# BichenWuUCB/squeezeDet

Hardware: AMD Instinct MI355X
Metric: images/sec SqueezeDet 1242x375 inference (higher is better)
Workload: dtype f16; 1 GPU; squeezeDet fp16 inference, batch=32 per GPU, synthetic 1242x375 images (4 distinct batches in rotation), full hot path (forward + interpret_output + filter_prediction + filtered rows to pinned host memory), inputs resident in HBM; 2 batches in flight (consecutive steps alternate between 2 HIP streams); global_batch=32, parallelism=dp1 (independent image shards, no collective)

## Files before the change

squeezedet_amd/csrc/chain.hip:

```cpp
#include "conv_common.h"
#include "chain.h"
#include "filter_body.h"

namespace sqdet {

namespace {

constexpr int CROWS = 8, CCOLS = 16;
constexpr int CHP = (CROWS + 2) * (CCOLS + 2);
constexpr int CCHUNK = CHP * 64;
constexpr int STAGE_B = 12288;
constexpr int NIMG = 2;

struct ChainGeom {
  int nch, nsq, nb1, nb3, chain, base3, per3, nstages;
};

__host__ __device__ inline ChainGeom chain_geom(int s, int e1, int e3, int s2) {
  ChainGeom g;
  g.nch = (s * 2 + 63) / 64;
  g.nsq = s2 / 16;
  g.nb1 = e1 / 64;
  g.nb3 = e3 / 64;
  g.chain = s2 > 0 ? 1 : 0;
  g.base3 = g.nb1 * (1 + g.chain);
  g.per3 = 3 * g.nch + g.chain;
  g.nstages = g.base3 + g.nb3 * g.per3;
  return g;
}

struct ChainArgs {
  const void* sq_in;
  void* sq_out;
  void* y;
  const unsigned char* stream;
  const float *b1, *b3, *bs2;
  int N, H, W, S, E1, E3, S2;
  int tiles_x, tiles_y;
  int nb1, nb3, nstages;
  unsigned in_bytes, out_bytes, y_bytes;
  int per_xcd;
  ChainRide ride;
};

__device__ __forceinline__ void glds16(unsigned voff, const unsigned char* sbase, unsigned lds_dst) {
  asm volatile("s_mov_b32 m0, %2\n\ts_nop 0\n\tglobal_load_lds_dwordx4 %0, %1" ::"v"(voff), "s"(sbase), "s"(lds_dst) : "memory", "m0");
}

#ifdef SQDET_CHAIN_TIMELINE
__device__ unsigned long long g_chain_tl[4096 * 8];
#define CTL(k) do { ctl[k] = wall_clock64(); } while (0)
#else
#define CTL(k) do {} while (0)
#endif

template <int N>
__device__ __forceinline__ void vm_wait() {
  asm volatile("s_waitcnt vmcnt(%0)" ::"n"(N) : "memory");
}

__device__ __forceinline__ i32x4 pack8(const f32x4& a, const f32x4& b) {
  f16x8 h = {(f16)a[0], (f16)a[1], (f16)a[2], (f16)a[3], (f16)b[0], (f16)b[1], (f16)b[2], (f16)b[3]};
  return __builtin_bit_cast(i32x4, h);
}

__device__ __forceinline__ f32x4 relu4(f32x4 v) {
  v[0] = fmaxf(v[0], 0.f); v[1] = fmaxf(v[1], 0.f); v[2] = fmaxf(v[2], 0.f); v[3] = fmaxf(v[3], 0.f);
  return v;
}

template <int NCH, int NSQ, bool WY, int RING, int DBG = 0>
__global__ __launch_bounds__(512, 2) void fire_chain(ChainArgs a) {
  using T = f16;
  constexpr int LOOK = RING - 2;
  constexpr int TH = (NSQ + 1) / 2;
  extern __shared__ __attribute__((aligned(16))) unsigned char lds[];
  const int lane = threadIdx.x & 63;
  const int wave = __builtin_amdgcn_readfirstlane((int)(threadIdx.x >> 6));
  const int pg = wave & 3, h = wave >> 2;
  const int j = lane & 15, g = lane >> 4;
#ifdef SQDET_CHAIN_TIMELINE
  unsigned long long ctl[8] = {0, 0, 0, 0, 0, 0, 0, 0};
#endif
  CTL(0);

  if ((int)(blockIdx.x >> 3) >= a.per_xcd) {
    const int rider = (int)((blockIdx.x >> 3) - a.per_xcd) * 8 + (int)(blockIdx.x & 7);
    FastLds<512>& fs = *reinterpret_cast<FastLds<512>*>(lds);
    for (int im = rider; im < a.ride.nimg; im += a.ride.nriders) {
      filter_one_image<true, f16, 512>(a.ride.fa, a.ride.da, a.ride.img0 + im, fs);
      __syncthreads();
    }
    return;
  }
  int b = (int)((blockIdx.x & 7) * a.per_xcd + (blockIdx.x >> 3));
  const int npairs = (a.N + 1) >> 1;
  if (b >= npairs * a.tiles_x * a.tiles_y) return;
  const int tx = b % a.tiles_x; b /= a.tiles_x;
  const int ty = b % a.tiles_y;
  const int np = b / a.tiles_y;
  const int oy0 = ty * CROWS, ox0 = tx * CCOLS;

  unsigned char* ring = lds;
  unsigned char* stile = lds + RING * STAGE_B;
  unsigned char* xch = stile + NIMG * NCH * CCHUNK;
  float* bl = reinterpret_cast<float*>(xch + (NSQ > 0 ? 32768 : 0));
  const unsigned ring_addr = (unsigned)(uintptr_t)(__attribute__((address_space(3))) unsigned char*)ring;

  constexpr int NP = NCH * 4;
  constexpr int SIT = (NIMG * CHP * NP + 511) / 512;
  i32x4 sv[SIT];
  {
    const int s_pieces = a.S * 2 / 16;
    const __amdgpu_buffer_rsrc_t rin = __builtin_amdgcn_make_buffer_rsrc(const_cast<void*>(a.sq_in), 0, a.in_bytes, 0x00020000);
    constexpr unsigned OOB = 0xfffffff0u;
#pragma unroll
    for (int it = 0; it < SIT; ++it) {
      const int idx = it * 512 + (int)threadIdx.x;
      const int im = idx / (CHP * NP);
      const int rem = idx - im * (CHP * NP);
      const int P = rem / NP, q = rem - P * NP;
      const int r = P / (CCOLS + 2), c = P - r * (CCOLS + 2);
      const int iy = oy0 - 1 + r, ix = ox0 - 1 + c;
      const int n = np * 2 + im;
      const bool ok = idx < NIMG * CHP * NP && q < s_pieces && n < a.N && iy >= 0 && iy < a.H && ix >= 0 && ix < a.W;
      const unsigned off = ok ? (unsigned)((((n * a.H + iy) * a.W + ix) * a.S) * 2 + q * 16) : OOB;
      sv[it] = __builtin_amdgcn_raw_buffer_load_b128(rin, off, 0, 0);
    }
  }

  const unsigned voff1 = (unsigned)(wave * 1024 + lane * 16), voff2 = voff1 + 8192;
  const unsigned char* sp = a.stream;
  const unsigned m0_lo = ring_addr + (unsigned)wave * 1024;
  unsigned m0n = m0_lo;
  auto refill = [&]() {
    if constexpr (DBG >= 2) return;
    glds16(voff1, sp, m0n);
    if (h == 0) glds16(voff2, sp, m0n + 8192);
    sp += STAGE_B;
    m0n = m0n + STAGE_B == m0_lo + RING * STAGE_B ? m0_lo : m0n + STAGE_B;
  };
#pragma unroll
  for (int s = 0; s < LOOK; ++s) refill();
  CTL(1);

  {
#pragma unroll
    for (int it = 0; it < SIT; ++it) {
      const int idx = it * 512 + (int)threadIdx.x;
      const int im = idx / (CHP * NP);
      const int rem = idx - im * (CHP * NP);
      const int P = rem / NP, q = rem - P * NP;
      if (idx < NIMG * CHP * NP)
        *reinterpret_cast<i32x4*>(stile + (im * NCH + (q >> 2)) * CCHUNK + P * 64 + (((q & 3) ^ ((P >> 1) & 3)) << 4)) = sv[it];
    }
    const int nbias = a.E1 + a.E3 + a.S2;
    for (int i = threadIdx.x; i < nbias; i += 512)
      bl[i] = i < a.E1 ? a.b1[i] : (i < a.E1 + a.E3 ? a.b3[i - a.E1] : a.bs2[i - a.E1 - a.E3]);
  }
  __syncthreads();
  CTL(2);

  const int img = pg >> 1, r0 = (pg & 1) * 4;
  const unsigned char* simg = stile + img * NCH * CCHUNK;
  auto load_b = [&](int c, int rr, int dx) {
    const int P = (r0 + rr) * (CCOLS + 2) + j + dx;
    return *reinterpret_cast<const i32x4*>(simg + c * CCHUNK + P * 64 + ((g ^ ((P >> 1) & 3)) << 4));
  };
  unsigned cbo = 0, nbo = STAGE_B;
  auto lda = [&](unsigned bo, int f) {
    return *reinterpret_cast<const i32x4*>(ring + bo + f * 1024 + lane * 16);
  };
  int ks = 0, ep_ks = -100;
  auto sync = [&](bool lds_writes) {
    bool st = false;
    if constexpr (WY) { st = (ks - ep_ks) < LOOK; ++ks; }
    if constexpr (DBG < 1) {
      if (h == 0) { if (st) vm_wait<2 * (LOOK - 1) + 4>(); else vm_wait<2 * (LOOK - 1)>(); }
      else { if (st) vm_wait<(LOOK - 1) + 4>(); else vm_wait<(LOOK - 1)>(); }
    }
    if (lds_writes) asm volatile("s_waitcnt lgkmcnt(0)" ::: "memory");
    if constexpr (DBG < 3) __builtin_amdgcn_s_barrier();
    asm volatile("" ::: "memory");
  };
  auto next_buf = [&]() {
    cbo = nbo;
    nbo = nbo + STAGE_B == RING * STAGE_B ? 0 : nbo + STAGE_B;
  };

  f32x4 accs[TH > 0 ? TH : 1][4];
#pragma unroll
  for (int t = 0; t < (TH > 0 ? TH : 1); ++t)
#pragma unroll
    for (int m = 0; m < 4; ++m) accs[t][m] = f32x4{0.f, 0.f, 0.f, 0.f};

  const int ctot = a.E1 + a.E3;
  const __amdgpu_buffer_rsrc_t ry = __builtin_amdgcn_make_buffer_rsrc(a.y, 0, WY ? a.y_bytes : 0u, 0x00020000);
  const int n_img = np * 2 + img;
  const int ox = ox0 + j;
  const bool col_ok = ox < a.W && n_img < a.N;

  i32x4 an[2];
  sync(false);
  CTL(3);
  refill();
#pragma unroll
  for (int n = 0; n < 2; ++n) an[n] = lda(0, 2 * h + n);

  auto finish_block = [&](f32x4 (&acc)[4][2], int cc0) {
    i32x4 bf[4];
    {
      const f32x4 bias0 = *reinterpret_cast<const f32x4*>(bl + cc0 + h * 32 + g * 8);
      const f32x4 bias1 = *reinterpret_cast<const f32x4*>(bl + cc0 + h * 32 + g * 8 + 4);
#pragma unroll
      for (int m = 0; m < 4; ++m) bf[m] = pack8(relu4(acc[m][0] + bias0), relu4(acc[m][1] + bias1));
    }
    if (WY) {
#pragma unroll
      for (int m = 0; m < 4; ++m) {
        const int oy = oy0 + r0 + m;
        const bool ok = col_ok && oy < a.H;
        const unsigned off = ok ? (unsigned)((((n_img * a.H + oy) * a.W + ox) * ctot + cc0 + h * 32 + g * 8) * 2) : 0xfffffff0u;
        __builtin_amdgcn_raw_buffer_store_b128(bf[m], ry, off, 0, 0);
      }
      ep_ks = ks;
    }
    if constexpr (NSQ > 0) {
      i32x4 fr[2][TH];
#pragma unroll
      for (int u = 0; u < 2; ++u)
#pragma unroll
        for (int i = 0; i < TH; ++i) {
          const int t = min(h * TH + i, NSQ - 1);
          fr[u][i] = lda(cbo, u * NSQ + t);
        }
#pragma unroll
      for (int m = 0; m < 4; ++m)
        *reinterpret_cast<i32x4*>(xch + (wave * 4 + m) * 1024 + lane * 16) = bf[m];
      sync(true);
      i32x4 bx[2][4];
#pragma unroll
      for (int u = 0; u < 2; ++u)
#pragma unroll
        for (int m = 0; m < 4; ++m) bx[u][m] = *reinterpret_cast<const i32x4*>(xch + ((pg + 4 * u) * 4 + m) * 1024 + lane * 16);
#pragma unroll
      for (int n = 0; n < 2; ++n) an[n] = lda(nbo, 2 * h + n);
#pragma unroll
      for (int u = 0; u < 2; ++u) {
#pragma unroll
        for (int i = 0; i < TH; ++i) {
          if (NSQ % 2 == 0 || h * TH + i < NSQ) {
#pragma unroll
            for (int m = 0; m < 4; ++m) mma16<T>(accs[i][m], fr[u][i], bx[u][m]);
          }
          if (u == 0 && i == 0) refill();
        }
      }
      next_buf();
    }
  };

  {
    i32x4 b1f[NCH][4];
#pragma unroll
    for (int c = 0; c < NCH; ++c)
#pragma unroll
      for (int m = 0; m < 4; ++m) b1f[c][m] = load_b(c, m + 1, 1);
#pragma unroll 1
    for (int blk = 0; blk < a.nb1; ++blk) {
      f32x4 acc[4][2];
#pragma unroll
      for (int m = 0; m < 4; ++m)
#pragma unroll
        for (int n = 0; n < 2; ++n) acc[m][n] = f32x4{0.f, 0.f, 0.f, 0.f};
      i32x4 ac[2];
#pragma unroll
      for (int n = 0; n < 2; ++n) ac[n] = an[n];
#pragma unroll
      for (int c = 0; c < NCH; ++c) {
        i32x4 nx[2];
        if (c + 1 < NCH) {
#pragma unroll
          for (int n = 0; n < 2; ++n) nx[n] = lda(cbo, (c + 1) * 4 + 2 * h + n);
        } else {
          sync(false);
#pragma unroll
          for (int n = 0; n < 2; ++n) nx[n] = lda(nbo, 2 * h + n);
        }
#pragma unroll
        for (int m = 0; m < 4; ++m) {
#pragma unroll
          for (int n = 0; n < 2; ++n) mma16<T>(acc[m][n], ac[n], b1f[c][m]);
          if (c + 1 == NCH && m == 2 * h) refill();
        }
#pragma unroll
        for (int n = 0; n < 2; ++n) ac[n] = nx[n];
      }
#pragma unroll
      for (int n = 0; n < 2; ++n) an[n] = ac[n];
      next_buf();
      finish_block(acc, blk * 64);
    }
  }

  CTL(4);
  i32x4 B[6][3];
#pragma unroll
  for (int rr = 0; rr < 2; ++rr)
#pragma unroll
    for (int dx = 0; dx < 3; ++dx) B[rr][dx] = load_b(0, rr, dx);
#pragma unroll 1
  for (int blk = 0; blk < a.nb3; ++blk) {
    f32x4 acc[4][2];
#pragma unroll
    for (int m = 0; m < 4; ++m)
#pragma unroll
      for (int n = 0; n < 2; ++n) acc[m][n] = f32x4{0.f, 0.f, 0.f, 0.f};
    i32x4 ac[2];
#pragma unroll
    for (int n = 0; n < 2; ++n) ac[n] = an[n];
#pragma unroll
    for (int c = 0; c < NCH; ++c) {
#pragma unroll
      for (int dy = 0; dy < 3; ++dy) {
        if (DBG >= 4 && blk > 0) {
        } else if (dy == 0) {
#pragma unroll
          for (int rr = 2; rr < 5; ++rr)
#pragma unroll
            for (int dx = 0; dx < 3; ++dx) B[rr][dx] = load_b(c, rr, dx);
        } else if (dy == 1) {
#pragma unroll
          for (int dx = 0; dx < 3; ++dx) B[5][dx] = load_b(c, 5, dx);
        } else {
#pragma unroll
          for (int rr = 0; rr < 2; ++rr)
#pragma unroll
            for (int dx = 0; dx < 3; ++dx) B[rr][dx] = load_b((c + 1) % NCH, rr, dx);
        }
#pragma unroll
        for (int dx = 0; dx < 3; ++dx) {
          i32x4 nx[2];
          if (DBG >= 5 && blk > 0) {
            nx[0] = ac[1]; nx[1] = ac[0];
            if (dx == 2) sync(false);
          } else if (dx < 2) {
#pragma unroll
            for (int n = 0; n < 2; ++n) nx[n] = lda(cbo, (dx + 1) * 4 + 2 * h + n);
          } else {
            sync(false);
#pragma unroll
            for (int n = 0; n < 2; ++n) nx[n] = lda(nbo, 2 * h + n);
          }
#pragma unroll
          for (int m = 0; m < 4; ++m) {
#pragma unroll
            for (int n = 0; n < 2; ++n) mma16<T>(acc[m][n], ac[n], B[m + dy][dx]);
            if (dx == 2 && m == 2 * h) refill();
          }
#pragma unroll
          for (int n = 0; n < 2; ++n) ac[n] = nx[n];
        }
        next_buf();
      }
    }
#pragma unroll
    for (int n = 0; n < 2; ++n) an[n] = ac[n];
    if constexpr (DBG >= 6) {
#pragma unroll
      for (int m = 0; m < 4; ++m)
#pragma unroll
        for (int n = 0; n < 2; ++n) accs[0][m] += acc[m][n];
      next_buf();
    } else {
      finish_block(acc, a.E1 + blk * 64);
    }
  }
  CTL(5);
  vm_wait<0>();
  CTL(6);

  if constexpr (NSQ > 0) {
    T* so = reinterpret_cast<T*>(a.sq_out);
    const float* bs = bl + a.E1 + a.E3;
#pragma unroll
    for (int m = 0; m < 4; ++m) {
      const int oy = oy0 + r0 + m;
      if (col_ok && oy < a.H) {
        T* dst = so + ((size_t)(n_img * a.H + oy) * a.W + ox) * a.S2 + g * 4 * NSQ;
#pragma unroll
        for (int i = 0; i < TH; ++i) {
          const int t = h * TH + i;
          if (t < NSQ) {
            const f32x4 bias = *reinterpret_cast<const f32x4*>(bs + g * 4 * NSQ + t * 4);
            store4<T>(dst + t * 4, relu4(accs[i][m] + bias));
          }
        }
      }
    }
  }
#ifdef SQDET_CHAIN_TIMELINE
  CTL(7);
  if (threadIdx.x == 0 && blockIdx.x < 4096) {
#pragma unroll
    for (int k = 0; k < 8; ++k) g_chain_tl[(size_t)blockIdx.x * 8 + k] = ctl[k];
  }
#endif
}

__global__ void chain_pack_kernel(const float* __restrict__ w1, const float* __restrict__ w3, const float* __restrict__ ws2,
                                  f16* __restrict__ out, int S, int E1, int E3, int S2, ChainGeom gm, size_t total) {
  for (size_t idx = (size_t)blockIdx.x * blockDim.x + threadIdx.x; idx < total; idx += (size_t)gridDim.x * blockDim.x) {
    size_t t = idx;
    const int e = t % 8; t /= 8;
    const int lane = t % 64; t /= 64;
    const int tile = t % 4; t /= 4;
    const int slot = t % 3; t /= 3;
    const int stage = (int)t;
    const int i = lane & 15, g = lane >> 4;
    int kind, blk, r;
    int cc0 = 0;
    if (stage < gm.base3) {
      blk = stage / (1 + gm.chain);
      r = stage - blk * (1 + gm.chain);
      kind = r == 0 ? 0 : 2;
      cc0 = blk * 64;
    } else {
      const int k2 = stage - gm.base3;
      blk = k2 / gm.per3;
      r = k2 - blk * gm.per3;
      kind = r < 3 * gm.nch ? 1 : 2;
      cc0 = E1 + blk * 64;
    }
    const float* src = kind == 0 ? w1 : (kind == 1 ? w3 : ws2);
    if (!src) continue;
    float v = 0.f;
    if (kind == 2) {
      const int f = slot * 4 + tile;
      if (f < 2 * gm.nsq) {
        const int u = f / gm.nsq, tt = f - u * gm.nsq;
        const int co = (i >> 2) * 4 * gm.nsq + tt * 4 + (i & 3);
        const int ci = cc0 + u * 32 + g * 8 + e;
        v = ws2[(size_t)ci * S2 + co];
      }
    } else {
      const int co = blk * 64 + (tile >> 1) * 32 + (i >> 2) * 8 + (tile & 1) * 4 + (i & 3);
      if (kind == 0) {
        const int ci = slot * 32 + g * 8 + e;
        if (slot < gm.nch && ci < S) v = w1[(size_t)ci * E1 + co];
      } else {
        const int c = r / 3, dy = r - c * 3;
        const int ci = c * 32 + g * 8 + e;
        if (ci < S) v = w3[((size_t)(dy * 3 + slot) * S + ci) * E3 + co];
      }
    }
    out[idx] = (f16)v;
  }
}

struct ChainSArgs {
  const void* sq_in;
  void* sq_out;
  const unsigned char* stream;
  const float *b1, *b3, *bs2;
  int N, H, W, S, E1, E3, S2;
  int tiles_x, tiles_y, ntiles, nquads;
  int nb1, nb3;
  unsigned in_bytes;
};

constexpr int CS_TILES = 4;
constexpr int CS_LW = 24;
constexpr int CS_TILE_B = (CROWS + 2) * CS_LW * 64;

template <int NSQ>
__global__ __launch_bounds__(512, 2) void fire_chain_stream(ChainSArgs a) {
  using T = f16;
  constexpr int F1 = 4 + 2 * NSQ;
  constexpr int F3 = 36 + 2 * NSQ;
  constexpr int NP = 4;
  constexpr int SIT = (CHP * NP + 127) / 128;
  extern __shared__ __attribute__((aligned(16))) unsigned char lds[];
  const int lane = threadIdx.x & 63;
  const int wave = __builtin_amdgcn_readfirstlane((int)(threadIdx.x >> 6));
  const int j = lane & 15, g = lane >> 4;
  const int nfrag = a.nb1 * F1 + a.nb3 * F3;
  unsigned char* wres = lds;
  unsigned char* stile = lds + (size_t)nfrag * 1024;
  float* bl = reinterpret_cast<float*>(stile + CS_TILES * CS_TILE_B);

// ... 135 lines not shown
#pragma unroll
      for (int m = 0; m < 4; ++m) Bc[m] = load_b(m, 0);
#pragma unroll
      for (int tt = 0; tt < 4; ++tt) ac[tt] = wfrag(f0 + tt);
#pragma unroll
      for (int tap = 0; tap < 9; ++tap) {
        i32x4 Bn[4], an[4];
        if (tap + 1 < 9) {
          const int dy = (tap + 1) / 3, dx = (tap + 1) % 3;
#pragma unroll
          for (int m = 0; m < 4; ++m) Bn[m] = load_b(m + dy, dx);
#pragma unroll
          for (int tt = 0; tt < 4; ++tt) an[tt] = wfrag(f0 + (tap + 1) * 4 + tt);
        }
#pragma unroll
        for (int m = 0; m < 4; ++m)
#pragma unroll
          for (int tt = 0; tt < 4; ++tt) mma16<T>(acc[m][tt], ac[tt], Bc[m]);
        __builtin_amdgcn_sched_barrier(0);
        if (tap + 1 < 9) {
#pragma unroll
          for (int m = 0; m < 4; ++m) Bc[m] = Bn[m];
#pragma unroll
          for (int tt = 0; tt < 4; ++tt) ac[tt] = an[tt];
        }
      }
      finish_block(acc, a.E1 + blk * 64, f0 + 36);
    }
    {
      const float* bs = bl + a.E1 + a.E3;
#pragma unroll
      for (int m = 0; m < 4; ++m) {
        const int oy = oy0 + r0 + m;
        if (col_ok && oy < a.H) {
          T* dst = so + ((size_t)(n_img * a.H + oy) * a.W + ox) * a.S2 + g * 4 * NSQ;
#pragma unroll
          for (int tq = 0; tq < NSQ; ++tq) {
            const f32x4 bias = *reinterpret_cast<const f32x4*>(bs + g * 4 * NSQ + tq * 4);
            store4<T>(dst + tq * 4, relu4(accs[tq][m] + bias));
          }
        }
      }
    }
    __syncthreads();
  }
}

bool fire_chain_stream_shape(int s, int e1, int e3, int s2) {
  return s > 0 && s <= 32 && s % 8 == 0 && e1 % 64 == 0 && e3 % 64 == 0 && e1 > 0 && e3 > 0 && (s2 == 16 || s2 == 32 || s2 == 48) &&
         (size_t)((e1 / 64) * (4 + s2 / 8) + (e3 / 64) * (36 + s2 / 8)) * 1024 + CS_TILES * CS_TILE_B + (size_t)(e1 + e3 + s2) * 4 <= 160 * 1024;
}

template <int NSQ>
int launch_chain_stream(const ChainSArgs& a, hipStream_t st) {
  const size_t lds = (size_t)(a.nb1 * (4 + 2 * NSQ) + a.nb3 * (36 + 2 * NSQ)) * 1024 + CS_TILES * CS_TILE_B + (size_t)(a.E1 + a.E3 + a.S2) * 4;
  static PerDevice once;
  SQDET_CHECK_HIP(once.run([] { return hipFuncSetAttribute(reinterpret_cast<const void*>(&fire_chain_stream<NSQ>),
                                                           hipFuncAttributeMaxDynamicSharedMemorySize, 160 * 1024); }));
  int grid = cu_count();
  if (grid > (a.nquads + 7) / 8 * 8) grid = (a.nquads + 7) / 8 * 8;
  hipLaunchKernelGGL((fire_chain_stream<NSQ>), dim3((unsigned)grid), dim3(512), lds, st, a);
  SQDET_CHECK_HIP(hipGetLastError());
  return SQDET_OK;
}

constexpr size_t chain_lds_bytes(int nch, int nsq, int ring, int nbias) {
  return (size_t)ring * STAGE_B + (size_t)NIMG * nch * CCHUNK + (nsq > 0 ? 32768 : 0) + (size_t)nbias * 4;
}
constexpr int chain_ring(int nch, int nsq) { return chain_lds_bytes(nch, nsq, 6, 768 + 96) <= 160 * 1024 ? 6 : 4; }

template <int NCH, int NSQ, bool WY>
int launch_chain(const ChainArgs& a, hipStream_t st) {
  constexpr int RG = chain_ring(NCH, NSQ);
  const size_t lds = chain_lds_bytes(NCH, NSQ, RG, a.E1 + a.E3 + a.S2);
  static PerDevice once;
  SQDET_CHECK_HIP(once.run([] { return hipFuncSetAttribute(reinterpret_cast<const void*>(&fire_chain<NCH, NSQ, WY, RG>),
                                                           hipFuncAttributeMaxDynamicSharedMemorySize, 160 * 1024); }));
  const int wgs = ((a.N + 1) / 2) * a.tiles_x * a.tiles_y;
  ChainArgs& am = const_cast<ChainArgs&>(a);
  am.per_xcd = (wgs + 7) / 8;
  const int riders_per_xcd = a.ride.nimg > 0 ? (a.ride.nriders + 7) / 8 : 0;
  const dim3 grid((unsigned)(8 * (am.per_xcd + riders_per_xcd)));
  static_assert(sizeof(FastLds<512>) <= RG * STAGE_B, "the rider's state lives in the ring's LDS");
#ifdef SQDET_CHAIN_DBG
  if constexpr (NCH == 3 && NSQ == 6 && !WY) {
    const int d = tune(TUNE_DBG);
    static bool dbg_attr = false;
    if (!dbg_attr) {
      (void)hipFuncSetAttribute(reinterpret_cast<const void*>(&fire_chain<NCH, NSQ, WY, RG, 1>), hipFuncAttributeMaxDynamicSharedMemorySize, 160 * 1024);
      (void)hipFuncSetAttribute(reinterpret_cast<const void*>(&fire_chain<NCH, NSQ, WY, RG, 2>), hipFuncAttributeMaxDynamicSharedMemorySize, 160 * 1024);
      (void)hipFuncSetAttribute(reinterpret_cast<const void*>(&fire_chain<NCH, NSQ, WY, RG, 3>), hipFuncAttributeMaxDynamicSharedMemorySize, 160 * 1024);
      (void)hipFuncSetAttribute(reinterpret_cast<const void*>(&fire_chain<NCH, NSQ, WY, RG, 4>), hipFuncAttributeMaxDynamicSharedMemorySize, 160 * 1024);
      (void)hipFuncSetAttribute(reinterpret_cast<const void*>(&fire_chain<NCH, NSQ, WY, RG, 5>), hipFuncAttributeMaxDynamicSharedMemorySize, 160 * 1024);
      (void)hipFuncSetAttribute(reinterpret_cast<const void*>(&fire_chain<NCH, NSQ, WY, RG, 6>), hipFuncAttributeMaxDynamicSharedMemorySize, 160 * 1024);
      dbg_attr = true;
    }
    switch (d) {
      case 1: hipLaunchKernelGGL((fire_chain<NCH, NSQ, WY, RG, 1>), grid, dim3(512), lds, st, a); return SQDET_OK;
      case 2: hipLaunchKernelGGL((fire_chain<NCH, NSQ, WY, RG, 2>), grid, dim3(512), lds, st, a); return SQDET_OK;
      case 3: hipLaunchKernelGGL((fire_chain<NCH, NSQ, WY, RG, 3>), grid, dim3(512), lds, st, a); return SQDET_OK;
      case 4: hipLaunchKernelGGL((fire_chain<NCH, NSQ, WY, RG, 4>), grid, dim3(512), lds, st, a); return SQDET_OK;
      case 5: hipLaunchKernelGGL((fire_chain<NCH, NSQ, WY, RG, 5>), grid, dim3(512), lds, st, a); return SQDET_OK;
      case 6: hipLaunchKernelGGL((fire_chain<NCH, NSQ, WY, RG, 6>), grid, dim3(512), lds, st, a); return SQDET_OK;
      default: break;
    }
  }
#endif
  hipLaunchKernelGGL((fire_chain<NCH, NSQ, WY, RG>), grid, dim3(512), lds, st, a);
  SQDET_CHECK_HIP(hipGetLastError());
  return SQDET_OK;
}

template <int NCH, bool WY>
int dispatch_chain_nsq(const ChainArgs& a, int nsq, hipStream_t st) {
  if (nsq == 0) { if constexpr (WY) return launch_chain<NCH, 0, true>(a, st); }
  if constexpr (NCH == 1) {
    switch (nsq) {
      case 1: return launch_chain<NCH, 1, WY>(a, st);
      case 2: return launch_chain<NCH, 2, WY>(a, st);
      case 3: return launch_chain<NCH, 3, WY>(a, st);
      default: break;
    }
  } else {
    switch (nsq) {
      case 3: return launch_chain<NCH, 3, WY>(a, st);
      case 4: return launch_chain<NCH, 4, WY>(a, st);
      case 6: return launch_chain<NCH, 6, WY>(a, st);
      default: break;
    }
  }
  set_error("fire_chain: unsupported next-squeeze width");
  return SQDET_EUNSUPPORTED;
}

}

bool fire_chain_eligible(int s, int e1, int e3, int s2, int dtype) {
  if (dtype != SQDET_F16 || conv_algo() != 0) return false;
  if (s <= 0 || s % 8 != 0 || s > 96) return false;
  if (e1 <= 0 || e3 <= 0 || e1 % 64 != 0 || e3 % 64 != 0) return false;
  if (!(s2 == 0 || s2 == 16 || s2 == 32 || s2 == 48 || s2 == 64 || s2 == 96)) return false;
  const ChainGeom g = chain_geom(s, e1, e3, s2);
  if (g.nch < 1 || g.nch > 3) return false;
  if (e1 + e3 + s2 > 768 + 96) return false;
  return chain_lds_bytes(g.nch, g.nsq, chain_ring(g.nch, g.nsq), e1 + e3 + s2) <= 160 * 1024;
}

}

using namespace sqdet;

extern "C" size_t sqdet_fire_chain_stream_bytes(int s1x1, int e1x1, int e3x3, int next_s1x1, int dtype) {
  if (!fire_chain_eligible(s1x1, e1x1, e3x3, next_s1x1, dtype)) return 0;
  return (size_t)(chain_geom(s1x1, e1x1, e3x3, next_s1x1).nstages + 5) * STAGE_B;
}

extern "C" int sqdet_fire_chain_pack(const float* w_e1_hwio, const float* w_e3_hwio, const float* w_next_s_hwio,
                                     void* stream_buf, int s1x1, int e1x1, int e3x3, int next_s1x1, int dtype,
                                     sqdet_stream_t stream) {
  SQDET_REQUIRE(stream_buf, "fire_chain_pack: null stream buffer");
  SQDET_UNSUPPORTED(!fire_chain_eligible(s1x1, e1x1, e3x3, next_s1x1, dtype), "fire_chain_pack: shape/dtype not covered");
  const ChainGeom g = chain_geom(s1x1, e1x1, e3x3, next_s1x1);
  const size_t total = (size_t)g.nstages * STAGE_B / 2;
  const int blocks = (int)((total + 255) / 256 > 4096 ? 4096 : (total + 255) / 256);
  hipLaunchKernelGGL(chain_pack_kernel, dim3(blocks), dim3(256), 0, as_stream(stream), w_e1_hwio, w_e3_hwio,
                     next_s1x1 > 0 ? w_next_s_hwio : nullptr, (f16*)stream_buf, s1x1, e1x1, e3x3, next_s1x1, g, total);
  SQDET_CHECK_HIP(hipGetLastError());
  return SQDET_OK;
// ... 70 lines not shown
```

squeezedet_amd/csrc/conv.hip:

```cpp
#include <stdlib.h>
#include <string.h>

#include "conv_common.h"

namespace sqdet {

template <typename T, int MT, int NT>
__device__ __forceinline__ void conv_epilogue(const ConvArgs& a, f32x4 (&acc)[MT][NT], const int (&pix)[MT],
                                              const bool (&valid)[MT], int group, int g) {
  T* y = reinterpret_cast<T*>(a.y);
  const int cbase = group * (16 * NT) + g * (4 * NT);
#pragma unroll
  for (int n = 0; n < NT; ++n) {
    const int c = cbase + n * 4;
    if (c < a.Cout) {
      const f32x4 b = a.bias ? *reinterpret_cast<const f32x4*>(a.bias + c) : f32x4{0.f, 0.f, 0.f, 0.f};
#pragma unroll
      for (int m = 0; m < MT; ++m) {
        if (valid[m]) {
          f32x4 v = acc[m][n] + b;
          T* dst = y + (size_t)pix[m] * a.y_cstride + a.y_coffset + c;
          if (a.accum) {
            v[0] += (float)dst[0]; v[1] += (float)dst[1]; v[2] += (float)dst[2]; v[3] += (float)dst[3];
          }
// ... 282 lines not shown
  a.y_cstride = y_cstride; a.y_coffset = y_coffset; a.relu = relu;
  a.x_cstride = x_cstride; a.x_coffset = x_coffset; a.accum = accum;
  a.relu_of = relu_of;
  a.res = res == y ? nullptr : res;
  a.scores = nullptr; a.score_apg = 0; a.score_classes = 0;
  const bool plain = x_cstride == cin && x_coffset == 0 && !accum && bias != nullptr && !relu_of;
  SQDET_UNSUPPORTED(!plain && g.gather, "conv2d: channel-sliced / accumulating convs need Cin %% %d == 0", kg_);
  bool handled = false;
  int rc = SQDET_OK;
  if (a.res) {
    if (!g.gather) {
      rc = conv1x1_tile_launch(a, g, dtype, st, &handled);
      if (rc != SQDET_OK || handled) return rc;
    }
    const size_t esz = dtype_size(dtype);
    if (y_cstride == cout && y_coffset == 0)
      SQDET_CHECK_HIP(hipMemcpyAsync(y, a.res, (size_t)P * y_cstride * esz, hipMemcpyDeviceToDevice, st));
    else
      SQDET_CHECK_HIP(hipMemcpy2DAsync(static_cast<char*>(y) + y_coffset * esz, y_cstride * esz,
                                       static_cast<const char*>(a.res) + y_coffset * esz, y_cstride * esz, cout * esz, (size_t)P,
                                       hipMemcpyDeviceToDevice, st));
    a.res = nullptr;
  }
  if (plain || !g.gather) {
    rc = conv3x3_tile_launch(a, g, dtype, st, &handled);
    if (rc != SQDET_OK || handled) return rc;
  }
  if (plain) {
    rc = conv1x1_stream_launch(a, g, dtype, st, &handled);
    if (rc != SQDET_OK || handled) return rc;
  }
  if (plain) {
    rc = conv1x1_deepk_launch(a, g, dtype, st, &handled);
    if (rc != SQDET_OK || handled) return rc;
  }
  if (!g.gather) {
    rc = conv1x1_tile_launch(a, g, dtype, st, &handled);
    if (rc != SQDET_OK || handled) return rc;
  }
  rc = dtype == SQDET_F16 ? dispatch_mt<f16>(a, g.nt, g.gather, st) : dispatch_mt<float>(a, g.nt, g.gather, st);
  if (rc != SQDET_OK) return rc;
  SQDET_CHECK_HIP(hipGetLastError());
  return SQDET_OK;
}

int convdet_scored_launch(const void* x, const void* w_packed, const float* bias, void* preds, float* scores, int n, int h, int w,
                          int cin, int apg, int classes, int dtype, hipStream_t st) {
  SQDET_REQUIRE(x && w_packed && bias && preds && scores, "convdet: null pointer");
  SQDET_REQUIRE(n > 0 && h > 0 && w > 0 && cin > 0 && apg > 0 && classes > 0, "convdet: bad dims");
  const int cout = apg * (classes + 5);
  SQDET_UNSUPPORTED(conv_algo() != 0 || !convdet_score_supported(cout, apg, classes, dtype),
                    "convdet: the score epilogue needs float16, 9 anchors x (3 classes + 5) and conv_algo = auto");
  const ConvGeom g = conv_geom(3, cin, cout, dtype);
  SQDET_UNSUPPORTED(g.gather || !(g.nt == 5 && g.ngroups == 1 && g.nchunk >= 8 && g.nchunk % 4 == 0),
                    "convdet: Cin %d is not a split-K ConvDet shape", cin);
  ConvArgs a;
  a.x = x; a.wp = w_packed; a.bias = bias; a.y = preds;
  a.N = n; a.H = h; a.W = w; a.Cin = cin; a.Cout = cout; a.k = 3; a.stride = 1;
  a.pt = 1; a.pl = 1; a.Ho = h; a.Wo = w;
  const long P = (long)n * h * w;
  SQDET_UNSUPPORTED(P > (1L << 30), "convdet: more than 2^30 pixels");
  a.P = (int)P; a.ntiles = 0;
  a.nchunk = g.nchunk; a.steps = g.steps; a.ngroups = g.ngroups;
  a.y_cstride = cout; a.y_coffset = 0; a.relu = 0;
  a.x_cstride = cin; a.x_coffset = 0; a.accum = 0; a.relu_of = nullptr; a.res = nullptr;
  a.scores = scores; a.score_apg = apg; a.score_classes = classes;
  bool handled = false;
  const int rc = conv3x3_tile_launch(a, g, dtype, st, &handled);
  if (rc != SQDET_OK) return rc;
  SQDET_UNSUPPORTED(!handled, "convdet: the split-K kernel did not take this shape");
  return SQDET_OK;
}

static int g_conv_algo = -1;
int conv_algo() {
  if (g_conv_algo < 0) {
    const char* e = getenv("SQDET_CONV_ALGO");
    g_conv_algo = (e && !strcmp(e, "generic")) ? 1 : 0;
  }
  return g_conv_algo;
}
void set_conv_algo(int v) { g_conv_algo = v; }

static const char* const kTuneNames[] = {"c1_waves", "c1_mt", "c1_min_tiles", "fire_fuse", "stem_algo", "dbg", "g1_wr", "g1_mbw", "g1_ntw", "g1_ns", "conv_pool"};
constexpr int kNumTune = 11;
static int g_tune[kNumTune] = {0, 0, 0, 0, 0, 0, 0, 0, 0, 0, 1};
int tune(int which) { return g_tune[which]; }

}

using namespace sqdet;

extern "C" int sqdet_set_option(const char* name, int value) {
  SQDET_REQUIRE(name, "set_option: null name");
  if (!strcmp(name, "conv_algo")) {
    SQDET_REQUIRE(value == 0 || value == 1, "set_option: conv_algo must be 0 (auto) or 1 (generic kernels only)");
    set_conv_algo(value);
    return SQDET_OK;
  }
  for (int i = 0; i < kNumTune; ++i) {
    if (!strcmp(name, kTuneNames[i])) {
      g_tune[i] = value;
      return SQDET_OK;
    }
  }
  set_error("set_option: unknown option '%s'", name);
  return SQDET_EINVAL;
}

extern "C" size_t sqdet_conv_packed_bytes(int k, int cin, int cout, int dtype) {
  if (k <= 0 || cin <= 0 || cout <= 0 || (dtype != SQDET_F16 && dtype != SQDET_F32)) return 0;
  const ConvGeom g = conv_geom(k, cin, cout, dtype);
  return (size_t)g.ngroups * g.steps * g.nt * 1024;
}

extern "C" int sqdet_conv_pack_weights(const float* w_hwio_f32, void* packed, int k, int cin, int cout, int dtype,
                                       sqdet_stream_t stream) {
  SQDET_REQUIRE(w_hwio_f32 && packed, "pack_weights: null pointer");
  SQDET_REQUIRE(k > 0 && cin > 0 && cout > 0, "pack_weights: bad dims");
  SQDET_REQUIRE(dtype == SQDET_F16 || dtype == SQDET_F32, "pack_weights: bad dtype %d", dtype);
  const ConvGeom g = conv_geom(k, cin, cout, dtype);
  const size_t total = (size_t)g.ngroups * g.steps * g.nt * 64 * g.kg;
  const int blocks = (int)((total + 255) / 256 > 4096 ? 4096 : (total + 255) / 256);
  if (dtype == SQDET_F16)
    hipLaunchKernelGGL(pack_weights_kernel<f16>, dim3(blocks), dim3(256), 0, as_stream(stream), w_hwio_f32,
                       (f16*)packed, g.taps, g.kdim, cout, g.nchunk, g.nt, total);
  else
    hipLaunchKernelGGL(pack_weights_kernel<float>, dim3(blocks), dim3(256), 0, as_stream(stream), w_hwio_f32,
                       (float*)packed, g.taps, g.kdim, cout, g.nchunk, g.nt, total);
  SQDET_CHECK_HIP(hipGetLastError());
  return SQDET_OK;
}

extern "C" int sqdet_conv2d_nhwc_fwd(const void* x, const void* w_packed, const float* bias, void* y, int n, int h,
                                     int w, int cin, int cout, int k, int stride, int pad_mode, int relu, int dtype,
                                     int y_cstride, int y_coffset, sqdet_stream_t stream) {
  return conv2d_launch(x, w_packed, bias, y, n, h, w, cin, cout, k, stride, pad_mode, relu, dtype, y_cstride,
                       y_coffset, as_stream(stream));
}

extern "C" int sqdet_convdet_fwd(const void* x, const void* w_packed, const float* bias, void* preds, float* scores, int n, int h,
                                 int w, int cin, int anchors_per_grid, int classes, int dtype, sqdet_stream_t stream) {
  return convdet_scored_launch(x, w_packed, bias, preds, scores, n, h, w, cin, anchors_per_grid, classes, dtype, as_stream(stream));
}

extern "C" int sqdet_convdet_scores_supported(int cin, int anchors_per_grid, int classes, int dtype) {
  const int cout = anchors_per_grid * (classes + 5);
  if (conv_algo() != 0 || !convdet_score_supported(cout, anchors_per_grid, classes, dtype)) return 0;
  const ConvGeom g = conv_geom(3, cin, cout, dtype);
  return (!g.gather && g.nt == 5 && g.ngroups == 1 && g.nchunk >= 8 && g.nchunk % 4 == 0) ? 1 : 0;
}

extern "C" int sqdet_conv2d_res_nhwc_fwd(const void* x, const void* w_packed, const float* bias, const void* residual, void* y, int n,
                                         int h, int w, int cin, int cout, int k, int stride, int pad_mode, int relu, int dtype,
                                         int y_cstride, int y_coffset, sqdet_stream_t stream) {
  SQDET_REQUIRE(residual, "conv2d_res: null residual");
  return conv2d_launch_res(x, w_packed, bias, y, n, h, w, cin, cout, k, stride, pad_mode, relu, dtype, y_cstride, y_coffset, cin, 0, 1,
                           nullptr, residual, as_stream(stream));
}

extern "C" int sqdet_conv2d_add_nhwc_fwd(const void* x, const void* w_packed, const float* bias, void* y_inout, int n,
                                         int h, int w, int cin, int cout, int k, int stride, int pad_mode, int relu,
                                         int dtype, int y_cstride, int y_coffset, sqdet_stream_t stream) {
  return conv2d_launch_ex(x, w_packed, bias, y_inout, n, h, w, cin, cout, k, stride, pad_mode, relu, dtype, y_cstride,
                          y_coffset, cin, 0, 1, as_stream(stream));
}
```

squeezedet_amd/csrc/launch.h:

```cpp
#pragma once
#include "common.h"

namespace sqdet {

struct ConvArgs;

int conv_algo();
enum { TUNE_C1_WAVES = 0, TUNE_C1_MT = 1, TUNE_C1_MIN_TILES = 2, TUNE_FIRE_FUSE = 3, TUNE_STEM_ALGO = 4, TUNE_DBG = 5, TUNE_G1_WR = 6, TUNE_G1_MBW = 7, TUNE_G1_NTW = 8, TUNE_G1_NS = 9,
       TUNE_CONV_POOL = 10 };
int tune(int which);
int conv2d_launch(const void* x, const void* w_packed, const float* bias, void* y, int n, int h, int w, int cin,
                  int cout, int k, int stride, int pad_mode, int relu, int dtype, int y_cstride, int y_coffset,
                  hipStream_t st);
int conv2d_launch_ex(const void* x, const void* w_packed, const float* bias, void* y, int n, int h, int w, int cin,
                     int cout, int k, int stride, int pad_mode, int relu, int dtype, int y_cstride, int y_coffset,
                     int x_cstride, int x_coffset, int accum, hipStream_t st);
int conv2d_launch_masked(const void* x, const void* w_packed, const float* bias, void* y, int n, int h, int w, int cin,
                         int cout, int k, int stride, int pad_mode, int relu, int dtype, int y_cstride, int y_coffset,
                         int x_cstride, int x_coffset, int accum, const void* relu_of, hipStream_t st);
int convdet_scored_launch(const void* x, const void* w_packed, const float* bias, void* preds, float* scores, int n, int h, int w,
                          int cin, int apg, int classes, int dtype, hipStream_t st);
bool convdet_score_supported(int cout, int apg, int classes, int dtype);

int conv1x1_stream_launch(const ConvArgs& a, const ConvGeom& g, int dtype, hipStream_t st, bool* handled);
int conv1x1_tile_launch(const ConvArgs& a, const ConvGeom& g, int dtype, hipStream_t st, bool* handled);
int conv1x1_deepk_launch(const ConvArgs& a, const ConvGeom& g, int dtype, hipStream_t st, bool* handled);
int conv3x3_tile_launch(const ConvArgs& a, const ConvGeom& g, int dtype, hipStream_t st, bool* handled);
int conv3x3_pool2_launch(const ConvArgs& a, const ConvGeom& g, int dtype, hipStream_t st, bool* handled, bool dry,
                         unsigned char* widx = nullptr);
bool conv2d_maxpool2_eligible(int n, int h, int w, int cin, int cout, int dtype);
int conv2d_maxpool2_launch(const void* x, const void* w_packed, const float* bias, void* y, int n, int h, int w, int cin, int cout,
                           int relu, int dtype, hipStream_t st, unsigned char* widx = nullptr);
bool conv3x3_pair_eligible(int n, int h, int w, int s, int e1, int e3, int dtype);
int conv3x3_pair_launch(const void* sq_in, const void* w3, const float* b3, const void* w1, const float* b1, void* y, int n, int h, int w,
                        int s, int e1, int e3, int dtype, hipStream_t st, bool* handled);

int maxpool_launch(const void* x, void* y, int n, int h, int w, int c, int k, int stride, int pad_mode, int dtype,
                   hipStream_t st);
int fold_bn_launch(const float* w, const float* cbias, const float* gamma, const float* beta, const float* mean,
                   const float* var, float eps, float* wf, float* bf, int k, int cin, int cout, hipStream_t st);

int stem_launch(const void* x, const void* w_packed, const float* bias, void* y, int n, int h, int w, int cout, int k,
                int conv_pad, int pool_pad, int dtype, int y_cstride, int y_coffset, hipStream_t st, bool* handled);
int stem_squeeze_launch(const void* x, const void* w_packed, const float* bias, const void* ws2_packed, const float* bs2,
                        void* s_out, int n, int h, int w, int cout, int k, int conv_pad, int pool_pad, int s2, int dtype,
                        hipStream_t st, bool* handled);
bool stem_squeeze_eligible(int h, int w, int cout, int k, int conv_pad, int pool_pad, int s2, int dtype, int n);

bool fire_fused_eligible(int cin, int s, int e1, int e3, int dtype);
int fire_fused_launch(const void* x, const void* ws, const float* bs, const void* w1, const float* b1, const void* w3,
                      const float* b3, void* y, int n, int h, int w, int cin, int s, int e1, int e3, int dtype,
                      hipStream_t st, bool* handled);
int fire_fused_launch_keep(const void* x, const void* ws, const float* bs, const void* w1, const float* b1, const void* w3,
                           const float* b3, void* sq_out, void* y, int n, int h, int w, int cin, int s, int e1, int e3, int dtype,
                           hipStream_t st, bool* handled);

bool fire_stream_eligible(int cin, int s, int e1, int e3, int dtype);
int fire_stream_launch_keep(const void* x, const void* ws, const float* bs, const void* w1, const float* b1, const void* w3,
                            const float* b3, void* sq_out, void* y, int n, int h, int w, int cin, int s, int e1, int e3, int dtype,
                            hipStream_t st, bool* handled);
int fire_stream_launch(const void* x, const void* ws, const float* bs, const void* w1, const float* b1, const void* w3,
                       const float* b3, void* y, int n, int h, int w, int cin, int s, int e1, int e3, int dtype,
                       hipStream_t st, bool* handled);
int fire_stream_launch_ex(const void* x, const void* ws, const float* bs, const void* w1, const float* b1, const void* w3,
                          const float* b3, void* y, int n, int h, int w, int cin, int s, int e1, int e3, int dtype,
                          int pool, hipStream_t st, bool* handled);
bool fire_expand_stream_eligible(int s, int e1, int e3, int dtype);
int fire_expand_stream_launch(const void* sq_in, const void* w1, const float* b1, const void* w3, const float* b3, void* y,
                              int n, int h, int w, int s, int e1, int e3, int dtype, int pool, hipStream_t st, bool* handled);
bool fire_squeeze_next_eligible(int cin, int s, int e1, int e3, int s2, int dtype);
int fire_squeeze_next_launch(const void* x, const void* ws, const float* bs, const void* w1, const float* b1, const void* w3,
                             const float* b3, const void* ws2, const float* bs2, void* s_out, int n, int h, int w, int cin,
                             int s, int e1, int e3, int s2, int dtype, hipStream_t st, bool* handled);
bool fire_expand_squeeze_next_eligible(int s, int e1, int e3, int s2, int pool, int dtype);
int fire_expand_squeeze_next_launch(const void* sq_in, const void* w1, const float* b1, const void* w3, const float* b3,
                                    const void* ws2, const float* bs2, void* s_out, int n, int h, int w, int s, int e1, int e3,
                                    int s2, int pool, int dtype, hipStream_t st, bool* handled);
int fire_dma_launch(const void* sq_in, const void* w1, const float* b1, const void* w3, const float* b3, const void* ws2,
                    const float* bs2, void* s_out, int n, int h, int w, int s, int e1, int e3, int s2, int pool, int dtype,
                    hipStream_t st, bool* handled);

bool fire_chain_eligible(int s, int e1, int e3, int s2, int dtype);

}
```

Baseline: 84010 images/s.

## Add paired-stage hand-over variant of fire_chain to halve ring barriers

Result: no change. 83990 images/s (median of 3 runs) (-0.0%).

```diff
diff --git a/squeezedet_amd/csrc/chain.hip b/squeezedet_amd/csrc/chain.hip
--- a/squeezedet_amd/csrc/chain.hip
+++ b/squeezedet_amd/csrc/chain.hip
@@ -69,10 +69,14 @@
   return v;
 }
 
-template <int NCH, int NSQ, bool WY, int RING, int DBG = 0>
-__global__ __launch_bounds__(512, 2) void fire_chain(ChainArgs a) {
+constexpr int PAIR_BEHIND = 1;
+constexpr int pair_wait(int h, int ne) { return PAIR_BEHIND * (2 - h) + 4 * ne; }
+
+template <int NCH, int NSQ, bool WY, int RING, int DBG, bool PAIR>
+__device__ __forceinline__ void fire_chain_body(const ChainArgs& a) {
   using T = f16;
-  constexpr int LOOK = RING - 2;
+  static_assert(!PAIR || RING == 6, "a paired hand-over needs the 6-stage ring");
+  constexpr int LOOK = PAIR ? 3 : RING - 2;
   constexpr int TH = (NSQ + 1) / 2;
   extern __shared__ __attribute__((aligned(16))) unsigned char lds[];
   const int lane = threadIdx.x & 63;
@@ -172,20 +176,43 @@
     return *reinterpret_cast<const i32x4*>(ring + bo + f * 1024 + lane * 16);
   };
   int ks = 0, ep_ks = -100;
-  auto sync = [&](bool lds_writes) {
-    bool st = false;
-    if constexpr (WY) { st = (ks - ep_ks) < LOOK; ++ks; }
-    if constexpr (DBG < 1) {
-      if (h == 0) { if (st) vm_wait<2 * (LOOK - 1) + 4>(); else vm_wait<2 * (LOOK - 1)>(); }
-      else { if (st) vm_wait<(LOOK - 1) + 4>(); else vm_wait<(LOOK - 1)>(); }
-    }
-    if (lds_writes) asm volatile("s_waitcnt lgkmcnt(0)" ::: "memory");
-    if constexpr (DBG < 3) __builtin_amdgcn_s_barrier();
-    asm volatile("" ::: "memory");
+  int odd = 1;
+  int ne = 0;
+  auto sync = [&](bool lds_writes, bool guard = false) {
+    if constexpr (PAIR) {
+      const bool ho = odd != 0;
+      if (ho) {
+        if constexpr (DBG < 1) {
+          if constexpr (WY) {
+            if (h == 0) { if (ne == 0) vm_wait<pair_wait(0, 0)>(); else if (ne == 1) vm_wait<pair_wait(0, 1)>(); else vm_wait<pair_wait(0, 2)>(); }
+            else { if (ne == 0) vm_wait<pair_wait(1, 0)>(); else if (ne == 1) vm_wait<pair_wait(1, 1)>(); else vm_wait<pair_wait(1, 2)>(); }
+            ne = 0;
+          } else {
+            if (h == 0) vm_wait<pair_wait(0, 0)>(); else vm_wait<pair_wait(1, 0)>();
+          }
+        }
+      }
+      if (lds_writes) asm volatile("s_waitcnt lgkmcnt(0)" ::: "memory");
+      if constexpr (DBG < 3) { if (ho || lds_writes || guard) __builtin_amdgcn_s_barrier(); }
+      asm volatile("" ::: "memory");
+      return ho;
+    } else {
+      bool st = false;
+      if constexpr (WY) { st = (ks - ep_ks) < LOOK; ++ks; }
+      if constexpr (DBG < 1) {
+        if (h == 0) { if (st) vm_wait<2 * (LOOK - 1) + 4>(); else vm_wait<2 * (LOOK - 1)>(); }
+        else { if (st) vm_wait<(LOOK - 1) + 4>(); else vm_wait<(LOOK - 1)>(); }
+      }
+      if (lds_writes) asm volatile("s_waitcnt lgkmcnt(0)" ::: "memory");
+      if constexpr (DBG < 3) __builtin_amdgcn_s_barrier();
+      asm volatile("" ::: "memory");
+      return true;
+    }
   };
   auto next_buf = [&]() {
     cbo = nbo;
     nbo = nbo + STAGE_B == RING * STAGE_B ? 0 : nbo + STAGE_B;
+    if constexpr (PAIR) odd ^= 1;
   };
 
   f32x4 accs[TH > 0 ? TH : 1][4];
@@ -204,6 +231,7 @@
   sync(false);
   CTL(3);
   refill();
+  if constexpr (PAIR) { refill(); odd = 0; }
 #pragma unroll
   for (int n = 0; n < 2; ++n) an[n] = lda(0, 2 * h + n);
 
@@ -224,6 +252,7 @@
         __builtin_amdgcn_raw_buffer_store_b128(bf[m], ry, off, 0, 0);
       }
       ep_ks = ks;
+      if constexpr (PAIR) ++ne;
     }
     if constexpr (NSQ > 0) {
       i32x4 fr[2][TH];
@@ -237,7 +266,7 @@
 #pragma unroll
       for (int m = 0; m < 4; ++m)
         *reinterpret_cast<i32x4*>(xch + (wave * 4 + m) * 1024 + lane * 16) = bf[m];
-      sync(true);
+      const bool ho = sync(true);
       i32x4 bx[2][4];
 #pragma unroll
       for (int u = 0; u < 2; ++u)
@@ -253,7 +282,7 @@
 #pragma unroll
             for (int m = 0; m < 4; ++m) mma16<T>(accs[i][m], fr[u][i], bx[u][m]);
           }
-          if (u == 0 && i == 0) refill();
+          if (i == 0 && ho && (u == 0 || PAIR)) refill();
         }
       }
       next_buf();
@@ -274,6 +303,7 @@
 #pragma unroll
         for (int n = 0; n < 2; ++n) acc[m][n] = f32x4{0.f, 0.f, 0.f, 0.f};
       i32x4 ac[2];
+      bool ho = false;
 #pragma unroll
       for (int n = 0; n < 2; ++n) ac[n] = an[n];
 #pragma unroll
@@ -283,7 +313,7 @@
 #pragma unroll
           for (int n = 0; n < 2; ++n) nx[n] = lda(cbo, (c + 1) * 4 + 2 * h + n);
         } else {
-          sync(false);
+          ho = sync(false, NSQ > 0);
 #pragma unroll
           for (int n = 0; n < 2; ++n) nx[n] = lda(nbo, 2 * h + n);
         }
@@ -291,7 +321,7 @@
         for (int m = 0; m < 4; ++m) {
 #pragma unroll
           for (int n = 0; n < 2; ++n) mma16<T>(acc[m][n], ac[n], b1f[c][m]);
-          if (c + 1 == NCH && m == 2 * h) refill();
+          if (c + 1 == NCH && ho && (m == 2 * h || (PAIR && m == 2 * h + 1))) refill();
         }
 #pragma unroll
         for (int n = 0; n < 2; ++n) ac[n] = nx[n];
@@ -341,14 +371,15 @@
 #pragma unroll
         for (int dx = 0; dx < 3; ++dx) {
           i32x4 nx[2];
+          bool ho = false;
           if (DBG >= 5 && blk > 0) {
             nx[0] = ac[1]; nx[1] = ac[0];
-            if (dx == 2) sync(false);
+            if (dx == 2) ho = sync(false);
           } else if (dx < 2) {
 #pragma unroll
             for (int n = 0; n < 2; ++n) nx[n] = lda(cbo, (dx + 1) * 4 + 2 * h + n);
           } else {
-            sync(false);
+            ho = sync(false);
 #pragma unroll
             for (int n = 0; n < 2; ++n) nx[n] = lda(nbo, 2 * h + n);
           }
@@ -356,7 +387,7 @@
           for (int m = 0; m < 4; ++m) {
 #pragma unroll
             for (int n = 0; n < 2; ++n) mma16<T>(acc[m][n], ac[n], B[m + dy][dx]);
-            if (dx == 2 && m == 2 * h) refill();
+            if (dx == 2 && ho && (m == 2 * h || (PAIR && m == 2 * h + 1))) refill();
           }
 #pragma unroll
           for (int n = 0; n < 2; ++n) ac[n] = nx[n];
@@ -406,6 +437,16 @@
     for (int k = 0; k < 8; ++k) g_chain_tl[(size_t)blockIdx.x * 8 + k] = ctl[k];
   }
 #endif
+}
+
+template <int NCH, int NSQ, bool WY, int RING, int DBG = 0>
+__global__ __launch_bounds__(512, 2) void fire_chain(ChainArgs a) {
+  fire_chain_body<NCH, NSQ, WY, RING, DBG, false>(a);
+}
+
+template <int NCH, int NSQ, bool WY, int DBG = 0>
+__global__ __launch_bounds__(512, 2) void fire_chain_pair(ChainArgs a) {
+  fire_chain_body<NCH, NSQ, WY, 6, DBG, true>(a);
 }
 
 __global__ void chain_pack_kernel(const float* __restrict__ w1, const float* __restrict__ w3, const float* __restrict__ ws2,
@@ -707,8 +748,35 @@
   const int riders_per_xcd = a.ride.nimg > 0 ? (a.ride.nriders + 7) / 8 : 0;
   const dim3 grid((unsigned)(8 * (am.per_xcd + riders_per_xcd)));
   static_assert(sizeof(FastLds<512>) <= RG * STAGE_B, "the rider's state lives in the ring's LDS");
+  if constexpr (RG == 6) {
+    if (tune(TUNE_CHAIN_PAIR) != 0) {
 #ifdef SQDET_CHAIN_DBG
-  if constexpr (NCH == 3 && NSQ == 6 && !WY) {
+      if constexpr (NCH == 2 && NSQ > 0 && !WY) {
+        static bool pdbg_attr = false;
+        if (!pdbg_attr) {
+          (void)hipFuncSetAttribute(reinterpret_cast<const void*>(&fire_chain_pair<NCH, NSQ, WY, 1>), hipFuncAttributeMaxDynamicSharedMemorySize, 160 * 1024);
+          (void)hipFuncSetAttribute(reinterpret_cast<const void*>(&fire_chain_pair<NCH, NSQ, WY, 2>), hipFuncAttributeMaxDynamicSharedMemorySize, 160 * 1024);
+          (void)hipFuncSetAttribute(reinterpret_cast<const void*>(&fire_chain_pair<NCH, NSQ, WY, 3>), hipFuncAttributeMaxDynamicSharedMemorySize, 160 * 1024);
+          pdbg_attr = true;
+        }
+        switch (tune(TUNE_DBG)) {
+          case 101: hipLaunchKernelGGL((fire_chain_pair<NCH, NSQ, WY, 1>), grid, dim3(512), lds, st, a); return SQDET_OK;
+          case 102: hipLaunchKernelGGL((fire_chain_pair<NCH, NSQ, WY, 2>), grid, dim3(512), lds, st, a); return SQDET_OK;
+          case 103: hipLaunchKernelGGL((fire_chain_pair<NCH, NSQ, WY, 3>), grid, dim3(512), lds, st, a); return SQDET_OK;
+          default: break;
+        }
+      }
+#endif
+      static PerDevice once_pair;
+      SQDET_CHECK_HIP(once_pair.run([] { return hipFuncSetAttribute(reinterpret_cast<const void*>(&fire_chain_pair<NCH, NSQ, WY>),
+                                                                    hipFuncAttributeMaxDynamicSharedMemorySize, 160 * 1024); }));
+      hipLaunchKernelGGL((fire_chain_pair<NCH, NSQ, WY>), grid, dim3(512), lds, st, a);
+      SQDET_CHECK_HIP(hipGetLastError());
+      return SQDET_OK;
+    }
+  }
+#ifdef SQDET_CHAIN_DBG
+  if constexpr ((NCH == 3 && NSQ == 6 && !WY) || (NCH == 2 && NSQ > 0 && !WY)) {
     const int d = tune(TUNE_DBG);
     static bool dbg_attr = false;
     if (!dbg_attr) {
diff --git a/squeezedet_amd/csrc/conv.hip b/squeezedet_amd/csrc/conv.hip
--- a/squeezedet_amd/csrc/conv.hip
+++ b/squeezedet_amd/csrc/conv.hip
@@ -388,9 +388,9 @@
 }
 void set_conv_algo(int v) { g_conv_algo = v; }
 
-static const char* const kTuneNames[] = {"c1_waves", "c1_mt", "c1_min_tiles", "fire_fuse", "stem_algo", "dbg", "g1_wr", "g1_mbw", "g1_ntw", "g1_ns", "conv_pool"};
-constexpr int kNumTune = 11;
-static int g_tune[kNumTune] = {0, 0, 0, 0, 0, 0, 0, 0, 0, 0, 1};
+static const char* const kTuneNames[] = {"c1_waves", "c1_mt", "c1_min_tiles", "fire_fuse", "stem_algo", "dbg", "g1_wr", "g1_mbw", "g1_ntw", "g1_ns", "conv_pool", "chain_pair"};
+constexpr int kNumTune = 12;
+static int g_tune[kNumTune] = {0, 0, 0, 0, 0, 0, 0, 0, 0, 0, 1, 1};
 int tune(int which) { return g_tune[which]; }
 
 }
diff --git a/squeezedet_amd/csrc/launch.h b/squeezedet_amd/csrc/launch.h
--- a/squeezedet_amd/csrc/launch.h
+++ b/squeezedet_amd/csrc/launch.h
@@ -7,7 +7,7 @@
 
 int conv_algo();
 enum { TUNE_C1_WAVES = 0, TUNE_C1_MT = 1, TUNE_C1_MIN_TILES = 2, TUNE_FIRE_FUSE = 3, TUNE_STEM_ALGO = 4, TUNE_DBG = 5, TUNE_G1_WR = 6, TUNE_G1_MBW = 7, TUNE_G1_NTW = 8, TUNE_G1_NS = 9,
-       TUNE_CONV_POOL = 10 };
+       TUNE_CONV_POOL = 10, TUNE_CHAIN_PAIR = 11 };
 int tune(int which);
 int conv2d_launch(const void* x, const void* w_packed, const float* bias, void* y, int n, int h, int w, int cin,
                   int cout, int k, int stride, int pad_mode, int relu, int dtype, int y_cstride, int y_coffset,
```
